# opensatelliteproject/xritdemod

Hardware: AMD Instinct MI355X
Metric: Msamples/s in -> soft-symbols/s out (LRIT 293 ksym/s chain); % HBM roofline (higher is better)
Workload: dtype f32

## Files before the change

### xritdemod_amd/csrc/agc.hip

```cpp
#include "kernels.h"

#include <cstdlib>
#include "scan.h"
#include "agc_wave.h"
#include "exact_walk.h"

namespace xrit {

struct AgcScanF {
    typedef AgcMap T;
    const float2 *x;
    float2 *y;
    const float *state_in;
    float *state_out;
    float rate, ref, maxg;
    long long n;
    int vec;

    __device__ T identity() const { return agc_identity(); }
    __device__ T combine(const T &lo, const T &hi) const { return agc_compose(lo, hi); }
    __device__ T reduce_run(long long i0, int cnt) const
    {
        T m = agc_identity();
        bool bad = false;
// ... 18 lines not shown
    {
        float g = agc_apply(pre, state_in[0]);
        if (cnt == SCAN_IPT && vec) {
            const float4 *xp = reinterpret_cast<const float4 *>(x + i0);
            float4 a = xp[0], b = xp[1], oa, ob;
            agc_step(a.x, a.y, g, rate, ref, maxg, oa.x, oa.y);
            agc_step(a.z, a.w, g, rate, ref, maxg, oa.z, oa.w);
            agc_step(b.x, b.y, g, rate, ref, maxg, ob.x, ob.y);
            agc_step(b.z, b.w, g, rate, ref, maxg, ob.z, ob.w);
            float4 *yp = reinterpret_cast<float4 *>(y + i0);
            yp[0] = oa;
            yp[1] = ob;
        } else {
            for (int k = 0; k < cnt; ++k) {
                float2 v = x[i0 + k];
                float yr, yi;
                agc_step(v.x, v.y, g, rate, ref, maxg, yr, yi);
                y[i0 + k] = make_float2(yr, yi);
            }
        }
        if (i0 + cnt == n) state_out[0] = g;
    }
};

__global__ void agc_serial_kernel(const float2 *x, float2 *y, const float *state_in, float *state_out,
                                  float rate, float ref, float maxg, long long n, int force)
{
    if (blockIdx.x != 0 || threadIdx.x != 0) return;
    if (!force && state_out[1] == 0.0f) return;
    float g = state_in[0];
    for (long long i = 0; i < n; ++i) {
        float2 v = x[i];
        float yr, yi;
        agc_step(v.x, v.y, g, rate, ref, maxg, yr, yi);
        y[i] = make_float2(yr, yi);
    }
    state_out[0] = g;
    state_out[1] = 2.0f;
}

__global__ void agc_begin_kernel(float *state_out)
{
    state_out[1] = 0.0f;
}

int AgcStage::init(float rate_, float reference, float gain0_, float max_gain)
{
    rate = rate_;
    ref = reference;
    maxg = max_gain;
    gain0 = gain0_;
    {
        int cus = 0, dev = 0;
        if (hipGetDevice(&dev) == hipSuccess && hipDeviceGetAttribute(&cus, hipDeviceAttributeMultiprocessorCount, dev) == hipSuccess && cus > 0)
            ex_walkers = 8 * cus;
        if (const char *e = getenv("XRIT_CX_WALKERS")) { const int v = atoi(e); if (v > 0) ex_walkers = v; }
        if (const char *e = getenv("XRIT_CX_MODE")) ex_mode = atoi(e) & 3;
    }
    XR_TRY(state.reserve(4 * sizeof(float)));
    float h[4] = {gain0_, 0.0f, gain0_, 0.0f};
    XR_HIP(hipMemcpy(state.p, h, sizeof h, hipMemcpyHostToDevice));
    if (!h_flag) XR_HIP(hipHostMalloc((void **)&h_flag, 64));
    *h_flag = 0.0f;
    cur = 0;
    return XRIT_OK;
}

__global__ void agc_reset_kernel(float *st, float g)
{
    st[0] = g; st[1] = 0.f; st[2] = g; st[3] = 0.f;
}

int AgcStage::reset(hipStream_t s)
{
    hipLaunchKernelGGL(agc_reset_kernel, dim3(1), dim3(1), 0, s, state.as<float>(), gain0);
    cur = 0;
    return XRIT_OK;
}

void AgcStage::release()
{
    state.release();
    aggs.release();
    joints.release();
    if (h_flag) { (void)hipHostFree(h_flag); h_flag = nullptr; }
}

int AgcStage::request_flag_at(const float *flag, hipStream_t s)
{
    XR_HIP(hipMemcpyAsync(h_flag, flag, sizeof(float), hipMemcpyDeviceToHost, s));
    return XRIT_OK;
}

int AgcStage::request_flag(hipStream_t s)
{
    XR_HIP(hipMemcpyAsync(h_flag, state.as<float>() + 2 * cur + 1, sizeof(float), hipMemcpyDeviceToHost, s));
    return XRIT_OK;
}

int AgcStage::run(const float2 *in, float2 *out, size_t n, hipStream_t s, Profiler *prof, bool use_exact)
{
    if (exact || use_exact) return run_exact(in, out, n, s, prof);
    if (n == 0) return XRIT_OK;
    float *sin_ = state.as<float>() + 2 * cur;
    float *sout = state.as<float>() + 2 * (cur ^ 1);
    int nb = scan_blocks((long long)n);
    XR_TRY(aggs.reserve((size_t)(nb + scan_blocks(nb) + 4) * sizeof(AgcMap)));
    const int vec = (((uintptr_t)in | (uintptr_t)out) & 15) == 0;
    AgcScanF f{in, out, sin_, sout, rate, ref, maxg, (long long)n, vec};
    {
        ProfScope ps(prof, "agc_reduce", s);
        hipLaunchKernelGGL(agc_begin_kernel, dim3(1), dim3(1), 0, s, sout);
        hipLaunchKernelGGL(scan_reduce_kernel<AgcScanF>, dim3(nb), dim3(SCAN_BLOCK), 0, s, f, (long long)n,
                           aggs.as<AgcMap>());
    }
    {
        ProfScope ps(prof, "agc_scan", s);
        scan_aggs_launch(f, aggs.as<AgcMap>(), nb, s);
    }
    {
        ProfScope ps(prof, "agc_apply", s);
        hipLaunchKernelGGL(scan_apply_kernel<AgcScanF>, dim3(nb), dim3(SCAN_BLOCK), 0, s, f, (long long)n,
                           aggs.as<AgcMap>());
        hipLaunchKernelGGL(agc_serial_kernel, dim3(1), dim3(1), 0, s, in, out, sin_, sout, rate, ref, maxg,
                           (long long)n, 0);
    }
    XR_HIP(hipGetLastError());
    cur ^= 1;
    return XRIT_OK;
}


constexpr int AGC_EX_WARM = 12288;
constexpr int AGC_EX_ROUNDS = 3;

__device__ __forceinline__ void agc_step_exact(float xr, float xi, float &g, float rate, float ref, float maxg, float &yr, float &yi)
{
    yr = xr * g;
    yi = xi * g;
    g += rate * (ref - ::sqrtf(yr * yr + yi * yi));
    if (maxg > 0.0f && g > maxg) g = maxg;
}

__device__ __forceinline__ float agx_scan(float d, float g0, float maxg, int mode, unsigned *lat)
{
    const int lane = threadIdx.x & 63;
    float gv = g0;
    if (mode & 2) {
        float gb = g0;
        int s = 0, seg = 0;
        bool done = false;
        for (; seg < 4 && !done; ++seg) {
            const bool in = lane >= s;
            const int og = xw::ord(gb);
            const int dG = in ? xw::ord(gb + d) - og : 0;
            const int S = xw::prefix(dG);
            const float gnext = xw::inv(og + S), gown = xw::inv(og + S - dG);
            float lg = gown + d;
            if (maxg > 0.0f && lg > maxg) lg = maxg;
            const unsigned long long bad = __builtin_amdgcn_ballot_w64(in && __float_as_uint(lg) != __float_as_uint(gnext));
            const int k = bad ? (int)__builtin_ctzll(bad) : 64;
            if (in && lane <= k) gv = gown;
            if (k >= 63) { done = true; break; }
            gb = xw::lane_of(lg, k);
            s = k + 1;
        }
// ... 88 lines not shown
    XR_TRY(aggs.reserve((size_t)(nb + scan_blocks(nb) + 4) * sizeof(AgcMap)));
    XR_TRY(joints.reserve((size_t)3 * W * sizeof(float2) + ((n >> 6) + 2) * sizeof(float2) + xw::NCNT * sizeof(unsigned)));
    AgcScanF f{in, out, sin_, sout, rate, ref, maxg, (long long)n, 0};
    {
        ProfScope ps(prof, "agc_reduce", s);
        hipLaunchKernelGGL(agc_begin_kernel, dim3(1), dim3(1), 0, s, sout);
        hipLaunchKernelGGL(scan_reduce_kernel<AgcScanF>, dim3(nb), dim3(SCAN_BLOCK), 0, s, f, (long long)n, aggs.as<AgcMap>());
    }
    {
        ProfScope ps(prof, "agc_scan", s);
        scan_aggs_launch(f, aggs.as<AgcMap>(), nb, s);
    }
    {
        ProfScope ps(prof, "agc_exact", s);
        xw::KArgs<AgcWalk> K{};
        xw::Args &A = K.a;
        A.x = in; A.y = out;
        A.js = joints.as<float2>(); A.je = A.js + W; A.used = A.je + W;
        A.bs = A.used + W;
        A.cnt = reinterpret_cast<unsigned *>(A.bs + (n >> 6) + 2);
        ex_cnt = A.cnt;
        A.n = (long long)n; A.Lw = (int)lw; A.H = AGC_EX_WARM; A.W = W;
        A.mode = ex_mode; A.prio = 1;
        K.p = AgcWalk::Par{aggs.as<AgcMap>(), sin_, sout, rate, ref, maxg};
        hipLaunchKernelGGL(xw::zero_kernel<AgcWalk>, dim3(1), dim3(64), 0, s, A.cnt, xw::NCNT);
        hipLaunchKernelGGL(xw::main_kernel<AgcWalk>, dim3(W), dim3(64), 0, s, K);
        hipLaunchKernelGGL(xw::used_kernel<AgcWalk>, dim3(div_up((size_t)W, 256)), dim3(256), 0, s, A);
        if (W > 1) {
            for (int r = 0; r < AGC_EX_ROUNDS; ++r) hipLaunchKernelGGL(xw::fix_kernel<AgcWalk>, dim3(W - 1), dim3(64), 0, s, K, 0);
            hipLaunchKernelGGL(xw::zero_kernel<AgcWalk>, dim3(1), dim3(64), 0, s, A.cnt, 1);
            hipLaunchKernelGGL(xw::fix_kernel<AgcWalk>, dim3(W - 1), dim3(64), 0, s, K, 1);
            hipLaunchKernelGGL(agc_exact_flag_kernel, dim3(1), dim3(1), 0, s, A.cnt, sout);
        }
        hipLaunchKernelGGL(agc_serial_exact_kernel, dim3(1), dim3(1), 0, s, in, out, sin_, sout, rate, ref, maxg, (long long)n);
    }
    XR_HIP(hipGetLastError());
    cur ^= 1;
    return XRIT_OK;
}

struct AgcRunF {
    typedef AgcMap T;
    __device__ T identity() const { return agc_identity(); }
    __device__ T combine(const T &lo, const T &hi) const { return agc_compose(lo, hi); }
};

template <int PL>
__global__ void __launch_bounds__(256) agc_apply_runs_kernel(const float2 *__restrict__ x, float2 *__restrict__ y,
                                                             const AgcMap *__restrict__ pre_run,
                                                             const float *__restrict__ state_in,
                                                             float *__restrict__ state_out, float rate, float ref,
                                                             float maxg, long long n)
{
    const int lane = threadIdx.x & 63;
    const long long run = (long long)blockIdx.x * 4 + (threadIdx.x >> 6);
    const long long i0 = run * (64 * PL) + (long long)lane * PL;
    int cnt = 0;
    if (i0 < n) cnt = (int)((n - i0) < PL ? (n - i0) : PL);
    float2 v[PL];
#pragma unroll
    for (int k = 0; k < PL; ++k) v[k] = k < cnt ? x[i0 + k] : make_float2(0.f, 0.f);
    AgcMap m = agc_identity();
#pragma unroll
    for (int k = 0; k < PL; ++k)
        if (k < cnt) m = agc_compose(m, agc_sample_map(v[k].x, v[k].y, rate, ref, maxg));
    const AgcMap ex = agc_wave_exclusive(m);
    if (cnt == 0) return;
    float g = agc_apply(agc_compose(pre_run[run], ex), state_in[0]);
#pragma unroll
    for (int k = 0; k < PL; ++k) {
        if (k < cnt) {
            float yr, yi;
            agc_step(v[k].x, v[k].y, g, rate, ref, maxg, yr, yi);
            y[i0 + k] = make_float2(yr, yi);
        }
    }
    if (i0 + cnt == n) state_out[0] = g;
}

constexpr int AGC_RUNS_PER_WAVE = 4;
template <int PL>
__global__ void __launch_bounds__(256) agc_run_maps_kernel(const float2 *__restrict__ x, AgcMap *__restrict__ maps,
                                                           float *__restrict__ state_out, float rate, float ref,
                                                           float maxg, long long n)
{
    const int lane = threadIdx.x & 63;
    const long long run0 = ((long long)blockIdx.x * 4 + (threadIdx.x >> 6)) * AGC_RUNS_PER_WAVE;
    float2 v[AGC_RUNS_PER_WAVE][PL];
#pragma unroll
    for (int r = 0; r < AGC_RUNS_PER_WAVE; ++r) {
        const long long i0 = (run0 + r) * (64 * PL) + (long long)lane * PL;
#pragma unroll
        for (int k = 0; k < PL; ++k) v[r][k] = x[min(i0 + k, n - 1)];
    }
    bool bad = false;
#pragma unroll
    for (int r = 0; r < AGC_RUNS_PER_WAVE; ++r) {
        const long long run = run0 + r;
        if (run * (64 * PL) >= n) break;
        const long long i0 = run * (64 * PL) + (long long)lane * PL;
        int cnt = 0;
        if (i0 < n) cnt = (int)((n - i0) < PL ? (n - i0) : PL);
        AgcMap m = agc_identity();
#pragma unroll
        for (int k = 0; k < PL; ++k) {
            if (k < cnt) {
                const AgcMap e = agc_sample_map(v[r][k].x, v[r][k].y, rate, ref, maxg);
                bad |= !(e.a >= 0.0f);
                m = agc_compose(m, e);
            }
        }
        m = agc_wave_total(m);
        if (lane == 0) maps[run] = m;
    }
    if (bad) state_out[1] = 1.0f;
}

int AgcStage::fused_reduce(const float2 *in, size_t n, int per_lane, hipStream_t s, Profiler *prof)
{
    AgcEpilogue epi{};
    XR_TRY(fused_begin(n, per_lane, s, &epi));
    if (n == 0) return XRIT_OK;
    if (per_lane != 3) { set_error("AGC: unsupported run shape %d", per_lane); return XRIT_E_INVALID; }
    const size_t rl = (size_t)64 * per_lane;
    const unsigned nr = div_up(n, rl);
    ProfScope ps(prof, "agc_reduce", s);
    hipLaunchKernelGGL(agc_run_maps_kernel<3>, dim3(div_up((size_t)nr, 4 * AGC_RUNS_PER_WAVE)), dim3(256), 0, s, in, epi.maps, epi.state_out,
                       rate, ref, maxg, (long long)n);
    XR_HIP(hipGetLastError());
    return XRIT_OK;
}

int AgcStage::fused_begin(size_t n, int per_lane, hipStream_t s, AgcEpilogue *epi)
{
    const size_t rl = (size_t)64 * per_lane;
    const int nr = (int)((n + rl - 1) / rl);
    XR_TRY(aggs.reserve((size_t)(nr + scan_blocks(nr) + 8) * sizeof(AgcMap)));
    float *sout = state.as<float>() + 2 * (cur ^ 1);
    hipLaunchKernelGGL(agc_begin_kernel, dim3(1), dim3(1), 0, s, sout);
    epi->maps = aggs.as<AgcMap>();
    epi->state_out = sout;
    epi->rate = rate;
    epi->ref = ref;
    epi->maxg = maxg;
    return XRIT_OK;
}

int AgcStage::fused_finish(const float2 *in, float2 *out, size_t n, int per_lane, hipStream_t s, Profiler *prof)
{
    if (n == 0) return XRIT_OK;
    float *sin_ = state.as<float>() + 2 * cur;
    float *sout = state.as<float>() + 2 * (cur ^ 1);
    const size_t rl = (size_t)64 * per_lane;
    const int nr = (int)((n + rl - 1) / rl);
    {
        ProfScope ps(prof, "agc_scan", s);
        scan_aggs_launch(AgcRunF{}, aggs.as<AgcMap>(), nr, s);
    }
    {
        ProfScope ps(prof, "agc_apply", s);
        const dim3 grid(div_up((size_t)nr, 4));
#define XR_AGC_APPLY(PL)                                                                                        \
    hipLaunchKernelGGL(agc_apply_runs_kernel<PL>, grid, dim3(256), 0, s, in, out, aggs.as<AgcMap>(), sin_, sout, \
                       rate, ref, maxg, (long long)n)
        switch (per_lane) {
        case 1: XR_AGC_APPLY(1); break;
        case 2: XR_AGC_APPLY(2); break;
        case 3: XR_AGC_APPLY(3); break;
        case 4: XR_AGC_APPLY(4); break;
        case 5: XR_AGC_APPLY(5); break;
        default: set_error("AGC: unsupported run shape %d", per_lane); return XRIT_E_INVALID;
        }
#undef XR_AGC_APPLY
        hipLaunchKernelGGL(agc_serial_kernel, dim3(1), dim3(1), 0, s, in, out, sin_, sout, rate, ref, maxg,
                           (long long)n, 0);
    }
    XR_HIP(hipGetLastError());
    cur ^= 1;
    return XRIT_OK;
}

int AgcStage::fused_scan(const float2 *in, float2 *fallback, size_t n, int per_lane, hipStream_t s, Profiler *prof,
                         AgcFill *fill)
{
    float *sin_ = state.as<float>() + 2 * cur;
    float *sout = state.as<float>() + 2 * (cur ^ 1);
    const size_t rl = (size_t)64 * per_lane;
    const int nr = (int)((n + rl - 1) / rl);
    {
        ProfScope ps(prof, "agc_scan", s);
        if (nr > 0) scan_aggs_launch(AgcRunF{}, aggs.as<AgcMap>(), nr, s);
        hipLaunchKernelGGL(agc_serial_kernel, dim3(1), dim3(1), 0, s, in, fallback, sin_, sout, rate, ref, maxg,
                           (long long)n, 0);
    }
    XR_HIP(hipGetLastError());
    fill->x = in;
    fill->pre_run = aggs.as<AgcMap>();
    fill->state_in = sin_;
    fill->state_out = sout;
    fill->rate = rate;
    fill->ref = ref;
    fill->maxg = maxg;
    fill->per_lane = per_lane;
    cur ^= 1;
    return XRIT_OK;
}

int AgcStage::exact_counters(unsigned *out8, hipStream_t s)
{
    for (int i = 0; i < 8; ++i) out8[i] = 0;
    if (!ex_cnt) return XRIT_OK;
    XR_HIP(hipMemcpyAsync(out8, ex_cnt, 8 * sizeof(unsigned), hipMemcpyDeviceToHost, s));
    XR_HIP(hipStreamSynchronize(s));
    return XRIT_OK;
}

int AgcStage::gain(float *g, hipStream_t s)
{
    XR_HIP(hipMemcpyAsync(g, state.as<float>() + 2 * cur, sizeof(float), hipMemcpyDeviceToHost, s));
    XR_HIP(hipStreamSynchronize(s));
    return XRIT_OK;
}

int AgcStage::fallback_flag(float *flag, hipStream_t s)
{
    XR_HIP(hipMemcpyAsync(flag, state.as<float>() + 2 * cur + 1, sizeof(float), hipMemcpyDeviceToHost, s));
    XR_HIP(hipStreamSynchronize(s));
    return XRIT_OK;
}

}
```

### xritdemod_amd/csrc/agc_wave.h

```cpp
#pragma once

#include <hip/hip_runtime.h>

#include "loop_core.h"

namespace xrit {

template <int CTRL> __device__ __forceinline__ float agc_dpp(float fill, float v)
{
    return __int_as_float(__builtin_amdgcn_update_dpp(__float_as_int(fill), __float_as_int(v), CTRL, 0xf, 0xf, false));
}

template <int SH> __device__ __forceinline__ AgcMap agc_row_shr(const AgcMap &v)
{
    AgcMap r;
    r.a = agc_dpp<0x110 + SH>(1.0f, v.a);
    r.b = agc_dpp<0x110 + SH>(0.0f, v.b);
    r.c = agc_dpp<0x110 + SH>(INFINITY, v.c);
    return r;
}

__device__ __forceinline__ AgcMap agc_row_scan(AgcMap v)
{
    v = agc_compose(agc_row_shr<1>(v), v);
    v = agc_compose(agc_row_shr<2>(v), v);
    v = agc_compose(agc_row_shr<4>(v), v);
    v = agc_compose(agc_row_shr<8>(v), v);
    return v;
}

__device__ __forceinline__ AgcMap agc_read_lane(const AgcMap &v, int lane)
{
    AgcMap r;
    r.a = __int_as_float(__builtin_amdgcn_readlane(__float_as_int(v.a), lane));
    r.b = __int_as_float(__builtin_amdgcn_readlane(__float_as_int(v.b), lane));
    r.c = __int_as_float(__builtin_amdgcn_readlane(__float_as_int(v.c), lane));
    return r;
}

__device__ __forceinline__ AgcMap agc_wave_total(const AgcMap &v)
{
    const AgcMap s = agc_row_scan(v);
    AgcMap t = agc_read_lane(s, 15);
    t = agc_compose(t, agc_read_lane(s, 31));
    t = agc_compose(t, agc_read_lane(s, 47));
    t = agc_compose(t, agc_read_lane(s, 63));
    return t;
}

__device__ __forceinline__ AgcMap agc_wave_exclusive(const AgcMap &v)
{
    const AgcMap s = agc_row_scan(v);
    const AgcMap t0 = agc_read_lane(s, 15), t1 = agc_read_lane(s, 31), t2 = agc_read_lane(s, 47);
    const int row = (threadIdx.x & 63) >> 4;
    AgcMap pre = agc_identity();
    if (row >= 1) pre = t0;
    if (row >= 2) pre = agc_compose(pre, t1);
    if (row >= 3) pre = agc_compose(pre, t2);
    return agc_compose(pre, agc_row_shr<1>(s));
}

}
```

### xritdemod_amd/csrc/demod.cpp

```cpp
#include "kernels.h"

#include <chrono>
#include <cmath>
#include <mutex>
#include <new>
#include <thread>
#include <vector>

namespace xrit {

static thread_local char g_err[512] = "";

void set_error(const char *fmt, ...)
{
    va_list ap;
    va_start(ap, fmt);
    vsnprintf(g_err, sizeof g_err, fmt, ap);
    va_end(ap);
}
const char *get_error() { return g_err; }

int select_device(int device)
{
    int count = 0;
// ... 347 lines not shown
    for (auto w : d->stream3) XR_HIP(hipStreamSynchronize(w));
    if (d->costas.job.n && d->pf_count > 0) {
        for (int i = 0; i < d->pf_count; ++i)
            if (d->pf[i].costas_begun && !d->pf[i].costas_finished) { bool redone = false; (void)d->costas.finish(d->pf[i].c_stream ? d->pf[i].c_stream : d->stream2, nullptr, &redone); }
    }
    d->pf_count = 0;
    d->last_fe_set = -1;
    XR_TRY(d->dec.reset(s));
    XR_TRY(d->rrc.reset(s));
    XR_TRY(d->agc.reset(s));
    XR_TRY(d->rtl.reset(s));
    XR_TRY(d->costas.reset(s));
    XR_TRY(d->clock.reset(s));
    d->poisoned = false;
    return XRIT_OK;
}

int xrit_build_experiments(void)
{
#ifdef XRIT_EXPERIMENTS
    return 1;
#else
    return 0;
#endif
}

void *xrit_demod_stream(xrit_demod *d) { return d ? (void *)d->stream : nullptr; }
float xrit_demod_sps(const xrit_demod *d) { return d ? d->sps : 0.f; }
int xrit_demod_decimator_ntaps(const xrit_demod *d) { return d ? d->dec_ntaps : 0; }

static int keep_stage(xrit_demod *d, int idx, const void *src, size_t n, hipStream_t s)
{
    if (!d->keep_stages) return XRIT_OK;
    XR_TRY(d->stage_buf[idx].reserve((n + 1) * sizeof(float2)));
    if (n) XR_HIP(hipMemcpyAsync(d->stage_buf[idx].p, src, n * sizeof(float2), hipMemcpyDeviceToDevice, s));
    d->stage_n[idx] = n;
    return XRIT_OK;
}

struct SliceIO {
    size_t length = 0;
    const float2 *rrc = nullptr;
    bool stat_ready = false;
    int set = 0;
    const float *agc_flag = nullptr;
    bool exact = false;
};

static bool front_exact_call(const xrit_demod *d, size_t n)
{
    if (d->cfg.front_exact == 2) return true;
    if (d->cfg.front_exact != 0) return false;
    const unsigned D = d->cfg.decimation;
    const double length = (double)(D > 1 ? n / D : n);
    return length / (double)d->sps < (double)d->clock.ov_min;
}

int xrit_demod_front_exact_for(const xrit_demod *d, size_t n)
{
    if (!d) return XRIT_E_INVALID;
    return front_exact_call(d, n) ? 1 : 0;
}

static int front_end(xrit_demod *d, const void *in, size_t n, int type, int set, hipStream_t s, Profiler *prof, SliceIO *io)
{
    io->set = set;
    const bool ex = front_exact_call(d, n);
    io->exact = ex;
    const unsigned D = d->cfg.decimation;
    if (type == XRIT_SAMPLE_U8IQ) {
        XR_TRY(d->bufR[set].reserve((n + 8) * sizeof(float2)));
        XR_TRY(d->rtl.run(in, d->bufR[set].as<float2>(), n, s, prof));
        in = d->bufR[set].p;
        type = XRIT_SAMPLE_FLOATIQ;
    }
    size_t length = n;
    if (D > 1) length = n / D;
    io->length = length;
    XR_TRY(d->bufA[set].reserve((length + 8) * sizeof(float2)));
    XR_TRY(d->bufB[set].reserve((length + 8) * sizeof(float2)));
    float2 *A = d->bufA[set].as<float2>(), *B = d->bufB[set].as<float2>();
    const float2 *cur = nullptr;
    const bool agc_fused = !ex && D > 1 && length > 0 && d->dec.agc_supported();
    if (D > 1) {
        AgcEpilogue epi{};
        if (agc_fused) XR_TRY(d->agc.fused_begin(length, d->dec.RC, s, &epi));
        XR_TRY(d->dec.run(in, type, A, length, s, prof, nullptr, 0, agc_fused ? &epi : nullptr, nullptr, ex));
        cur = A;
    } else if (type != XRIT_SAMPLE_FLOATIQ) {
        ProfScope ps(prof, "convert", s);
        XR_TRY(launch_convert(in, type, A, length, s));
        cur = A;
    } else {
        cur = reinterpret_cast<const float2 *>(in);
    }
    XR_TRY(keep_stage(d, 0, cur, length, s));
    const bool agc_in_rrc = agc_fused && !d->keep_stages && d->rrc.agc_fill_supported(d->dec.RC);
    const bool agc_in_rrc_d1 = !ex && !agc_fused && length > 0 && !d->keep_stages && d->rrc.agc_fill_supported(3);
    AgcFill fill{};
    float2 *Cfb = nullptr;
    if (agc_in_rrc || agc_in_rrc_d1) {
        XR_TRY(d->bufC[set].reserve((length + 8) * sizeof(float2)));
        Cfb = d->bufC[set].as<float2>();
        if (agc_in_rrc_d1) XR_TRY(d->agc.fused_reduce(cur, length, 3, s, prof));
        XR_TRY(d->agc.fused_scan(cur, Cfb, length, agc_in_rrc ? d->dec.RC : 3, s, prof, &fill));
    }
    else if (agc_fused) XR_TRY(d->agc.fused_finish(cur, B, length, d->dec.RC, s, prof));
    else XR_TRY(d->agc.run(cur, B, length, s, prof, ex));
    XR_TRY(keep_stage(d, 1, B, length, s));
    constexpr int SUB = 8;
    XR_TRY(d->stat[set].reserve(((length + SUB - 1) / SUB + 2) * sizeof(float2)));
    io->stat_ready = length > 0 && d->rrc.stat_supported(SUB) && d->costas.L % SUB == 0;
    const bool fill_on = agc_in_rrc || agc_in_rrc_d1;
    float2 *rrc_out = fill_on ? B : A;
    XR_TRY(d->rrc.run(fill_on ? Cfb : B, XRIT_SAMPLE_FLOATIQ, rrc_out, length, s, prof, io->stat_ready ? d->stat[set].as<float2>() : nullptr, SUB,
                      nullptr, fill_on ? &fill : nullptr, ex));
    XR_TRY(keep_stage(d, 2, rrc_out, length, s));
    io->rrc = rrc_out;
    io->agc_flag = d->agc.state.as<float>() + 2 * d->agc.cur + 1;
    return XRIT_OK;
}

static bool ov_call(xrit_demod *d, size_t n);

static int launch_prefetched(xrit_demod *d, xrit_demod::Prefetched &f, hipEvent_t after)
{
    XR_HIP(hipStreamWaitEvent(d->stream2, d->ev_ready, 0));
    if (after) XR_HIP(hipStreamWaitEvent(d->stream2, after, 0));
    if (d->last_fe_set >= 0) XR_HIP(hipStreamWaitEvent(d->stream2, d->ev_fe[d->last_fe_set], 0));
    const int set = d->next_set;
    d->next_set ^= 1;
    SliceIO io;
    Profiler *prof = d->prof.enabled ? &d->prof : nullptr;
    d->dec.prio = d->rrc.prio = ov_call(d, f.n) ? 1 : 0;
    int rc = front_end(d, f.samples, f.n, f.type, set, d->stream2, prof, &io);
    d->dec.prio = d->rrc.prio = 0;
    if (rc != XRIT_OK) { d->poisoned = true; return rc; }
    XR_HIP(hipEventRecord(d->ev_fe[set], d->stream2));
    d->last_fe_set = set;
    f.set = set;
    f.length = io.length; f.rrc = io.rrc; f.stat_ready = io.stat_ready; f.agc_flag = io.agc_flag; f.exact = io.exact;
    f.launched = true;
    return XRIT_OK;
}

static int costas_enqueue(xrit_demod *d, const SliceIO &io, hipStream_t s, Profiler *prof, float2 **slot_out)
{
    const size_t length = io.length;
    const int L = d->costas.L;
    float2 *slot = nullptr;
    XR_TRY(d->clock.input_slot(length, &slot, s));
    double2 *om = nullptr;
    if (length) om = d->clock.om_slot((int)((length + (size_t)L - 1) / (size_t)L), L);
    const double inv_sps = 1.0 / (double)d->sps;
    const float2 *stat = io.stat_ready ? d->stat[io.set].as<float2>() : nullptr;
    XR_TRY(d->costas.begin(io.rrc, slot, length, s, prof, stat, om, 0, inv_sps, io.exact));
    if (length) XR_TRY(d->clock.om_scan(s));
    if (length) XR_TRY(d->agc.request_flag_at(io.agc_flag, s));
    *slot_out = slot;
    return XRIT_OK;
}

static void set_relay_hook(xrit_demod *d, hipStream_t s)
{
    d->clock.before_relay = [d, s](int phase) -> int {
        if (phase == 0) {
            if (d->pf_count > 0 && !d->pf[0].launched) XR_HIP(hipEventRecord(d->ev_relay, s));
            return XRIT_OK;
        }
        if (d->pf_count > 0 && !d->pf[0].launched) {
            if (d->clock.trace_env) fprintf(stderr, "[xrit] the registered front end starts with the relay kernels%s\n", d->costas_idle ? ", its Costas loop behind it" : "");
            XR_TRY(launch_prefetched(d, d->pf[0], d->ev_relay));
            if (d->costas_idle) {
                xrit_demod::Prefetched &f = d->pf[0];
                SliceIO io;
                io.length = f.length; io.rrc = f.rrc; io.stat_ready = f.stat_ready; io.set = f.set; io.agc_flag = f.agc_flag; io.exact = f.exact;
                int rc = costas_enqueue(d, io, d->stream2, d->prof.enabled ? &d->prof : nullptr, &f.slot);
                if (rc != XRIT_OK) { d->poisoned = true; return rc; }
                XR_HIP(hipEventRecord(d->ev_costas, d->stream2));
                f.costas_begun = true;
// ... 872 lines not shown
```

### xritdemod_amd/csrc/fir.hip

```cpp
#include "kernels.h"

#include <cstdlib>
#include <new>
#include "agc_wave.h"

namespace xrit {

template <int TYPE> struct SampleLoad;
template <> struct SampleLoad<XRIT_SAMPLE_FLOATIQ> {
    static __device__ __forceinline__ float2 at(const void *p, size_t j) { return reinterpret_cast<const float2 *>(p)[j]; }
};
template <> struct SampleLoad<XRIT_SAMPLE_S16IQ> {
    static __device__ __forceinline__ float2 at(const void *p, size_t j)
    {
        short2 v = reinterpret_cast<const short2 *>(p)[j];
        return make_float2(v.x / 32768.f, v.y / 32768.f);
    }
};
template <> struct SampleLoad<XRIT_SAMPLE_S8IQ> {
    static __device__ __forceinline__ float2 at(const void *p, size_t j)
    {
        char2 v = reinterpret_cast<const char2 *>(p)[j];
        return make_float2(v.x / 128.f, v.y / 128.f);
    }
};

template <int APL>
__device__ __forceinline__ void fir_fill_through_agc(float2 *tile, const AgcFill &af, const float2 *__restrict__ hist,
                                                     int T, long long tile_start, int tile_len, long long n_in)
{
    constexpr int RL = 64 * APL;
    constexpr int MAXIT = 3;
    const int tid = threadIdx.x, nthr = blockDim.x;
    const int wave = tid >> 6, lane = tid & 63, nwaves = nthr >> 6;
    const long long t_end = tile_start + tile_len < n_in ? tile_start + tile_len : n_in;
    const long long first_run = (tile_start > 0 ? tile_start : 0) / RL;
    float2 v[MAXIT][APL];
    int cnt[MAXIT];
#pragma unroll
    for (int it = 0; it < MAXIT; ++it) {
        const long long rr = first_run + wave + (long long)it * nwaves;
        const long long i0 = rr * RL + (long long)lane * APL;
        cnt[it] = 0;
        if (rr * RL < t_end && i0 < n_in) cnt[it] = (int)((n_in - i0) < APL ? (n_in - i0) : APL);
#pragma unroll
        for (int k = 0; k < APL; ++k) v[it][k] = k < cnt[it] ? af.x[i0 + k] : make_float2(0.f, 0.f);
    }
    const float g0 = af.state_in[0];
#pragma unroll
    for (int it = 0; it < MAXIT; ++it) {
        const long long rr = first_run + wave + (long long)it * nwaves;
        if (rr * RL >= t_end) break;
        AgcMap m = agc_identity();
#pragma unroll
        for (int k = 0; k < APL; ++k)
            if (k < cnt[it]) m = agc_compose(m, agc_sample_map(v[it][k].x, v[it][k].y, af.rate, af.ref, af.maxg));
        const AgcMap ex = agc_wave_exclusive(m);
        float gg = agc_apply(agc_compose(af.pre_run[rr], ex), g0);
        const long long i0 = rr * RL + (long long)lane * APL;
#pragma unroll
        for (int k = 0; k < APL; ++k) {
            if (k < cnt[it]) {
                float yr, yi;
                agc_step(v[it][k].x, v[it][k].y, gg, af.rate, af.ref, af.maxg, yr, yi);
                const long long idx = i0 + k - tile_start;
                if (idx >= 0 && idx < tile_len) tile[idx] = make_float2(yr, yi);
                if (i0 + k == n_in - 1) af.state_out[0] = gg;
            }
        }
    }
    for (int idx = tid; idx < tile_len; idx += nthr) {
        const long long j = tile_start + idx;
        if (j < 0) {
            const long long hj = (T - 1) + j;
            tile[idx] = hj >= 0 ? hist[hj] : make_float2(0.f, 0.f);
        } else if (j >= n_in) {
            tile[idx] = make_float2(0.f, 0.f);
        }
    }
}

template <int TYPE>
__device__ __forceinline__ void fir_leave_history(const void *__restrict__ in, const float2 *__restrict__ hist_old,
                                                  float2 *__restrict__ hist_new, int T, long long n_in)
{
    for (int i = threadIdx.x; i < T - 1; i += blockDim.x) {
        const long long j = n_in - (T - 1) + i;
        float2 v;
        if (j >= 0) v = SampleLoad<TYPE>::at(in, (size_t)j);
        else {
            const long long hj = (T - 1) + j;
            v = hj >= 0 ? hist_old[hj] : make_float2(0.f, 0.f);
        }
        hist_new[i] = v;
    }
}

template <bool MF> __device__ __forceinline__ int fir_mf_pos(int q) { return MF ? q + 20 * (q / 80) : q; }

#ifndef XRIT_FE_PRIO
#define XRIT_FE_PRIO 1
#endif
template <int RC, bool PAD, int TYPE, int APL = 0, int TS = 0, int DS = 1, bool MF = false, bool EX = false>
__global__ void __launch_bounds__(256)
fir_decim_kernel(const void *__restrict__ in, const float2 *__restrict__ hist, float2 *__restrict__ out,
                 const float *__restrict__ g, int T, int D, int Wpad, long long n_out, long long n_in,
                 int tile_len, float2 *__restrict__ stat, int statL, AgcEpilogue agc, AgcFill af,
                 float2 *__restrict__ hist_new, const float *__restrict__ mfb = nullptr)
{
    if (statL >> 16) __builtin_amdgcn_s_setprio(XRIT_FE_PRIO);
    statL &= 0xffff;
    if (hist_new != nullptr && blockIdx.x == gridDim.x - 1 && (APL == 0 || af.state_out[1] != 0.0f))
        fir_leave_history<TYPE>(in, hist, hist_new, T, n_in);
    extern __shared__ __attribute__((aligned(16))) char smem_raw[];
    float2 *tile = reinterpret_cast<float2 *>(smem_raw);
    const int nthr = blockDim.x;
    const int tid = threadIdx.x;
    const long long OB = (long long)nthr * RC;
    const long long out_base = (long long)blockIdx.x * OB;
    const long long tile_start = out_base * D - (T - 1);

    if (APL > 0 && af.state_out[1] == 0.0f) {
        fir_fill_through_agc<(APL > 0 ? APL : 1)>(tile, af, hist, T, tile_start, tile_len, n_in);
    } else if (tile_start >= 0 && tile_start + tile_len <= n_in) {
        int idx = tid;
        if (TYPE == XRIT_SAMPLE_FLOATIQ && !PAD && !MF && (tile_start & 1) == 0 &&
            (reinterpret_cast<size_t>(in) & 15) == 0) {
            const float4 *in4 = reinterpret_cast<const float4 *>(reinterpret_cast<const float2 *>(in) + tile_start);
            float4 *tile4 = reinterpret_cast<float4 *>(tile);
            const int pairs = tile_len >> 1;
            int p = tid;
#ifndef XRIT_NO_LDS_DIRECT
            for (; p - (tid & 63) < pairs; p += nthr) {
                if (p < pairs)
                    __builtin_amdgcn_global_load_lds((const __attribute__((address_space(1))) void *)(in4 + p),
                                                     (__attribute__((address_space(3))) void *)(tile4 + (p - (tid & 63))), 16, 0, 0);
            }
            asm volatile("s_waitcnt vmcnt(0)" ::: "memory");
#endif
#define XR_TILE_BATCH4(U)                                                                   \
    for (; p + (U - 1) * nthr < pairs; p += U * nthr) {                                     \
        float4 v[U];                                                                        \
        _Pragma("unroll") for (int u = 0; u < U; ++u) v[u] = in4[p + u * nthr];             \
        _Pragma("unroll") for (int u = 0; u < U; ++u) tile4[p + u * nthr] = v[u];           \
    }
            XR_TILE_BATCH4(8)
            XR_TILE_BATCH4(4)
            XR_TILE_BATCH4(2)
            XR_TILE_BATCH4(1)
#undef XR_TILE_BATCH4
            idx = 2 * pairs + tid;
        }
#define XR_TILE_BATCH(U)                                                                                      \
    for (; idx + (U - 1) * nthr < tile_len; idx += U * nthr) {                                               \
        float2 v[U];                                                                                          \
        _Pragma("unroll") for (int u = 0; u < U; ++u)                                                         \
            v[u] = SampleLoad<TYPE>::at(in, (size_t)(tile_start + idx + u * nthr));                           \
        _Pragma("unroll") for (int u = 0; u < U; ++u) {                                                       \
            const int q = idx + u * nthr;                                                                     \
            tile[PAD ? q + q / D : fir_mf_pos<MF>(q)] = v[u];                                                 \
        }                                                                                                     \
    }
        XR_TILE_BATCH(8)
        XR_TILE_BATCH(4)
        XR_TILE_BATCH(2)
        XR_TILE_BATCH(1)
#undef XR_TILE_BATCH
    } else {
        for (int idx = tid; idx < tile_len; idx += nthr) {
            long long j = tile_start + idx;
            float2 v = make_float2(0.f, 0.f);
            if (j < 0) {
                long long hj = (T - 1) + j;
                if (hj >= 0) v = hist[hj];
            } else if (j < n_in) {
                v = SampleLoad<TYPE>::at(in, (size_t)j);
            }
            int pos = PAD ? idx + idx / D : fir_mf_pos<MF>(idx);
            tile[pos] = v;
        }
    }
    __syncthreads();
    if (APL > 0 && hist_new != nullptr && blockIdx.x == gridDim.x - 1 && af.state_out[1] == 0.0f) {
        for (int i = tid; i < T - 1; i += nthr) hist_new[i] = tile[(int)(n_in - (T - 1) + i - tile_start)];
    }

    float2 acc[RC];
#pragma unroll
    for (int c = 0; c < RC; ++c) acc[c] = make_float2(0.f, 0.f);

    const int lane_base = PAD ? tid * RC * (D + 1) : tid * RC * D;
    const float2 *w = tile + lane_base;
    if (MF) {
#ifdef XRIT_EXPERIMENTS
#include "../../experiments/csrc/fir_mfma_dec.inc"
#endif
    } else if (TS > 0) {
        typedef float v2f __attribute__((ext_vector_type(2)));
        constexpr int NP = (TS + 1) / 2;
        const unsigned long long *gp = reinterpret_cast<const unsigned long long *>(g);
        unsigned long long tp[NP > 0 ? NP : 1];
#pragma unroll
        for (int k = 0; k < NP; ++k) tp[k] = gp[k];
        v2f a[RC];
#pragma unroll
        for (int c = 0; c < RC; ++c) a[c] = (v2f){0.f, 0.f};
// ... 54 lines not shown
                float2 x = w[off + k];
#pragma unroll
                for (int c = 0; c < RC; ++c) {
                    float tp = g[c * Wpad + i + k];
                    acc[c].x = fmaf(tp, x.x, acc[c].x);
                    acc[c].y = fmaf(tp, x.y, acc[c].y);
                }
            }
            i += run;
            off += D + 1;
        }
    } else if (EX) {
        typedef float v2f __attribute__((ext_vector_type(2)));
        v2f a[RC][4];
#pragma unroll
        for (int c = 0; c < RC; ++c)
#pragma unroll
            for (int j = 0; j < 4; ++j) a[c][j] = (v2f){0.f, 0.f};
        for (int i = 0; i < Wpad; i += 4) {
            const float2 q0 = w[i], q1 = w[i + 1], q2 = w[i + 2], q3 = w[i + 3];
            const v2f x0 = {q0.x, q0.y}, x1 = {q1.x, q1.y}, x2 = {q2.x, q2.y}, x3 = {q3.x, q3.y};
#pragma unroll
            for (int c = 0; c < RC; ++c) {
                const float *gc = g + c * Wpad + i;
                const float t0 = gc[0], t1 = gc[1], t2 = gc[2], t3 = gc[3];
                const v2f p0 = x0 * t0, p1 = x1 * t1, p2 = x2 * t2, p3 = x3 * t3;
                a[c][0] = a[c][0] + p0;
                a[c][1] = a[c][1] + p1;
                a[c][2] = a[c][2] + p2;
                a[c][3] = a[c][3] + p3;
            }
        }
#pragma unroll
        for (int c = 0; c < RC; ++c) {
            const int sh = (c * D) & 3;
            v2f r;
            if (sh == 0) r = (a[c][0] + a[c][1]) + (a[c][2] + a[c][3]);
            else if (sh == 1) r = (a[c][1] + a[c][2]) + (a[c][3] + a[c][0]);
            else if (sh == 2) r = (a[c][2] + a[c][3]) + (a[c][0] + a[c][1]);
            else r = (a[c][3] + a[c][0]) + (a[c][1] + a[c][2]);
            acc[c] = make_float2(r.x, r.y);
        }
    } else {
        for (int i = 0; i < Wpad; i += 4) {
            float2 x0 = w[i], x1 = w[i + 1], x2 = w[i + 2], x3 = w[i + 3];
#pragma unroll
            for (int c = 0; c < RC; ++c) {
                const float *gc = g + c * Wpad + i;
                float t0 = gc[0], t1 = gc[1], t2 = gc[2], t3 = gc[3];
                acc[c].x = fmaf(t0, x0.x, acc[c].x);
                acc[c].y = fmaf(t0, x0.y, acc[c].y);
                acc[c].x = fmaf(t1, x1.x, acc[c].x);
                acc[c].y = fmaf(t1, x1.y, acc[c].y);
                acc[c].x = fmaf(t2, x2.x, acc[c].x);
                acc[c].y = fmaf(t2, x2.y, acc[c].y);
                acc[c].x = fmaf(t3, x3.x, acc[c].x);
                acc[c].y = fmaf(t3, x3.y, acc[c].y);
            }
        }
    }
    const long long m0 = out_base + (long long)tid * RC;
    {
        __syncthreads();
        float2 *ot = tile;
#pragma unroll
        for (int c = 0; c < RC; ++c) ot[tid * RC + c] = acc[c];
        __syncthreads();
        const long long left = n_out - out_base;
        const int cnt = left < OB ? (int)left : (int)OB;
        for (int k = tid; k < cnt; k += nthr) out[out_base + k] = ot[k];
    }
    if (!PAD && agc.maps != nullptr) {
        AgcMap v = agc_identity();
        bool bad = false;
#pragma unroll
        for (int c = 0; c < RC; ++c) {
            if (m0 + c < n_out) {
                AgcMap e = agc_sample_map(acc[c].x, acc[c].y, agc.rate, agc.ref, agc.maxg);
                bad |= !(e.a >= 0.0f);
                v = agc_compose(v, e);
            }
        }
        if (bad) agc.state_out[1] = 1.0f;
        v = agc_wave_total(v);
        const int lane = tid & 63;
        if (lane == 0 && m0 < n_out) agc.maps[m0 / (64 * RC)] = v;
    }
    if (stat != nullptr) {
        const float2 *ot = tile;
        if (statL == 8) {
            for (int i = tid; i < (int)OB; i += nthr) {
                const long long o = out_base + i;
                float sr = 0.f, si = 0.f;
                if (o < n_out) {
                    const float2 z = ot[i];
                    sr = z.x * z.x - z.y * z.y;
                    si = 2.0f * z.x * z.y;
                }
                sr += __int_as_float(__builtin_amdgcn_update_dpp(0, __float_as_int(sr), 0x111, 0xf, 0xf, true));
                si += __int_as_float(__builtin_amdgcn_update_dpp(0, __float_as_int(si), 0x111, 0xf, 0xf, true));
                sr += __int_as_float(__builtin_amdgcn_update_dpp(0, __float_as_int(sr), 0x112, 0xf, 0xf, true));
                si += __int_as_float(__builtin_amdgcn_update_dpp(0, __float_as_int(si), 0x112, 0xf, 0xf, true));
                sr += __int_as_float(__builtin_amdgcn_update_dpp(0, __float_as_int(sr), 0x114, 0xf, 0xf, true));
                si += __int_as_float(__builtin_amdgcn_update_dpp(0, __float_as_int(si), 0x114, 0xf, 0xf, true));
                if ((tid & 7) == 7 && o - 7 < n_out) stat[o >> 3] = make_float2(sr, si);
            }
        } else {
            const int runs = (int)(OB / statL);
            const int wave = tid >> 6, lane = tid & 63, nwaves = nthr >> 6;
            for (int j = wave; j < runs; j += nwaves) {
                const long long first = out_base + (long long)j * statL;
                if (first >= n_out) break;
                float sr = 0.f, si = 0.f;
                for (int i = lane; i < statL; i += 64) {
                    if (first + i < n_out) {
                        const float2 z = ot[j * statL + i];
                        sr += z.x * z.x - z.y * z.y;
                        si += 2.0f * z.x * z.y;
                    }
                }
                for (int off = 32; off > 0; off >>= 1) {
                    sr += __shfl_down(sr, off, 64);
                    si += __shfl_down(si, off, 64);
                }
                if (lane == 0) stat[first / statL] = make_float2(sr, si);
            }
        }
    }
}

#ifndef XRIT_POLY_THREADS
#define XRIT_POLY_THREADS 256
#endif
template <int DP, int PR, int NQ, int TYPE>
__global__ void __launch_bounds__(XRIT_POLY_THREADS)
fir_poly_kernel(const void *__restrict__ in, const float2 *__restrict__ hist, float2 *__restrict__ out,
                const float *__restrict__ hq , int T, long long n_out, long long n_in, int tile_len,
                float2 *__restrict__ hist_new)
{
    if (hist_new != nullptr && blockIdx.x == 0) fir_leave_history<TYPE>(in, hist, hist_new, T, n_in);
    extern __shared__ __attribute__((aligned(16))) char smem_raw[];
    float2 *tile = reinterpret_cast<float2 *>(smem_raw);
    const int tid = threadIdx.x, nthr = blockDim.x;
    const int OB = (nthr / DP) * PR;
    const unsigned per = gridDim.x >> 3;
    const long long tb = (long long)(blockIdx.x & 7) * per + (blockIdx.x >> 3);
    const long long out_base = tb * OB;
    if (out_base >= n_out) return;
    const long long tile_start = out_base * DP - (long long)(NQ * DP);

    if (TYPE == XRIT_SAMPLE_FLOATIQ && tile_start >= 0 && tile_start + tile_len <= n_in && (tile_start & 1) == 0 &&
        (reinterpret_cast<size_t>(in) & 15) == 0) {
        const float4 *in4 = reinterpret_cast<const float4 *>(reinterpret_cast<const float2 *>(in) + tile_start);
        float4 *tile4 = reinterpret_cast<float4 *>(tile);
        const int pairs = tile_len >> 1;
        constexpr int UF = (((NQ + (XRIT_POLY_THREADS / DP) * PR - 1) * DP + 2) / 2 + XRIT_POLY_THREADS - 1) / XRIT_POLY_THREADS;
#ifndef XRIT_NO_LDS_DIRECT
        for (int p = tid; p - (tid & 63) < pairs; p += nthr)
            if (p < pairs)
                __builtin_amdgcn_global_load_lds((const __attribute__((address_space(1))) void *)(in4 + p),
                                                 (__attribute__((address_space(3))) void *)(tile4 + (p - (tid & 63))), 16, 0, 0);
        asm volatile("s_waitcnt vmcnt(0)" ::: "memory");
        for (int p0 = pairs + tid; p0 < pairs; p0 += UF * nthr) {
#else
        for (int p0 = tid; p0 < pairs; p0 += UF * nthr) {
#endif
            float4 v[UF];
#pragma unroll
// ... 533 lines not shown
```

### xritdemod_amd/csrc/kernels.h

```cpp
#pragma once

#include <functional>

#include "common.h"
#include "loop_core.h"
#include "taps.h"

namespace xrit {

struct FirStage {
    int T = 0, D = 1, RC = 3, W = 0, Wpad = 0, threads = 256, tile_len = 0, cur = 0;
    bool pad = false;
    bool mfma_dec = false;
    bool no_static_dec = false, no_static_mf = false;
    int prio = 0;
    bool poly = false;
    bool exact = false, ex_pad = false;
    int ex_threads = 256, ex_opt = 2, ex_tile_len = 0;
    size_t ex_lds = 0;
    DevBuf rt;
    std::vector<float> taps_host;
    int set_exact(bool on);
#ifndef XRIT_POLY_PR
#define XRIT_POLY_PR 16
#endif
    static constexpr int POLY_PR = XRIT_POLY_PR, POLY_NQ = 32;
    size_t lds_bytes = 0;
    DevBuf g;
    DevBuf mfb;
    DevBuf hist[2];
    int init(const float *taps, int ntaps, int decim);
    int reset(hipStream_t s);
    void release();
    int run(const void *in, int sample_type, float2 *out, size_t n_out, hipStream_t s, Profiler *prof,
            float2 *stat = nullptr, int statL = 0, const struct AgcEpilogue *agc = nullptr,
            const struct AgcFill *fill = nullptr, bool use_exact = false);
    FirStage *twin = nullptr;
    bool last_twin = false;
    FirStage() = default;
    FirStage(const FirStage &) = delete;
    FirStage &operator=(const FirStage &) = delete;
    bool agc_fill_supported(int per_lane) const;
    bool stat_supported(int statL) const;
    bool agc_supported() const;
};

constexpr int AGC_RUN_MAX_PER_LANE = 5;
struct AgcFill {
    const float2 *x;
    const struct AgcMap *pre_run;
    const float *state_in;
    float *state_out;
    float rate, ref, maxg;
    int per_lane;
};
struct AgcEpilogue {
    struct AgcMap *maps;
    float *state_out;
    float rate, ref, maxg;
};

struct RtlIngestStage {
    float alpha = 0;
    DevBuf state;
    DevBuf aggs;
    int cur = 0;
    int init(float sample_rate);
    int reset(hipStream_t s);
    void release();
    int run(const void *in_u8, float2 *out, size_t n_complex, hipStream_t s, Profiler *prof);
};

struct AgcStage {
    float rate = 0, ref = 0, maxg = 0;
    DevBuf state;
    DevBuf aggs;
    int cur = 0;
    int init(float rate, float reference, float gain, float max_gain);
    int reset(hipStream_t s);
    float gain0 = 1.0f;
    void release();
    int run(const float2 *in, float2 *out, size_t n, hipStream_t s, Profiler *prof, bool use_exact = false);
    bool exact = false;
    DevBuf joints;
    int ex_walkers = 2048, ex_mode = 3;
    int run_exact(const float2 *in, float2 *out, size_t n, hipStream_t s, Profiler *prof);
    unsigned *ex_cnt = nullptr;
    int exact_counters(unsigned *out8, hipStream_t s);
    int fused_begin(size_t n, int per_lane, hipStream_t s, AgcEpilogue *epi);
    int fused_finish(const float2 *in, float2 *out, size_t n, int per_lane, hipStream_t s, Profiler *prof);
    int fused_reduce(const float2 *in, size_t n, int per_lane, hipStream_t s, Profiler *prof);
    int fused_scan(const float2 *in, float2 *fallback, size_t n, int per_lane, hipStream_t s, Profiler *prof, AgcFill *fill);
    int gain(float *g, hipStream_t s);
    int fallback_flag(float *flag, hipStream_t s);
    int request_flag(hipStream_t s);
    int request_flag_at(const float *flag, hipStream_t s);
    float requested_flag() const { return h_flag ? *h_flag : 0.0f; }
    float *h_flag = nullptr;
};

struct CostasStage {
    CostasGains gains{};
    int L = 256;
    int max_passes = 32;
    float trust = 1.0f, tol_phase = 1e-5f, tol_freq = 3e-8f;
    DevBuf state;
    DevBuf S, E, J, stat, sub, dlin, work, flags, counters, wsolve, rescue;
    bool model_step = true;
    float model_accept = 5e-3f;
    bool force_gated = false;
    int final_warm = 0;
    bool keep_spare = false, trace_env = false, no_serial_walk = false;
    int rescue_after = 32;
    long long rescue_max_samples = 4 << 20;
    unsigned rescues = 0;
    bool walked = false;
    int serial_rescue(hipStream_t s, Profiler *prof);
    unsigned *h_counters = nullptr;
    int cur = 0;
    int passes = 0;
    unsigned unconverged = 0;
    float max_residual = 0;
    int init(float loop_bw, int chain_len, int max_passes);
    int reset(hipStream_t s);
    void release();
    int run(const float2 *in, float2 *out, size_t n, hipStream_t s, Profiler *prof, const float2 *sub_ext = nullptr,
            double2 *om = nullptr, long long om_off = 0, double inv_sps = 0.0);
    int begin(const float2 *in, float2 *out, size_t n, hipStream_t s, Profiler *prof, const float2 *sub_ext,
              double2 *om, long long om_off, double inv_sps, bool use_exact = false);
    bool closed() const;
    int finish(hipStream_t s, Profiler *prof, bool *redone);
    int enqueue_passes(int count, hipStream_t s, Profiler *prof);
    int enqueue_final(hipStream_t s, Profiler *prof);
    struct Job {
        const float2 *in = nullptr; float2 *out = nullptr; size_t n = 0; int K = 0; int enqueued = 0;
        double2 *om = nullptr; long long om_off = 0; double inv_sps = 0;
        bool gated = false;
        bool rescued = false;
        bool exact = false;
        float model_accept = 0;
    } job;
    int batch = 4;
    int stable = 0, last_passes = -1;
    int get_state(float *phase, float *freq, hipStream_t s);
    bool exact = false;
    int ex_mode = 3;
    int ex_hist = -1;
    int ex_prio = 1;
    int ex_walkers = 2048;
    DevBuf xj, xbs, xcnt;
    unsigned *h_xcnt = nullptr;
    int ex_W = 0, ex_rounds = 0;
    bool ex_args_valid = false;
    unsigned ex_open = 0, ex_nonconverged = 0;
    unsigned long long ex_blocks = 0, ex_picard = 0, ex_segs = 0, ex_fallbacks = 0;
    int exact_plan(size_t n, int *Lw, int *W, int *H) const;
    int enqueue_exact(hipStream_t s, Profiler *prof);
    int finish_exact(hipStream_t s, Profiler *prof, bool *redone);
    int flip_phase(hipStream_t s);
};

int launch_loop_sincosf(const float *d_x, float *d_sin, float *d_cos, size_t n, hipStream_t s);

struct ClockStage {
    ClockPar par{};
    float sps = 0, mu0 = 0.5f;
    int NS = 64;
    int cu_count = 256;
    long long lds_per_cu = 160 * 1024;
    bool auto_ns = true;
    bool serial = false;
    int max_passes = 48, min_passes = 4;
// ... 184 lines not shown
```

Before: 154,300.

## Store per-lane AGC exclusive prefixes in reduce pass and reuse in RRC fill

The reduce pass (decimator epilogue or run-maps kernel) now keeps the intra-wave row scan and writes each lane's exclusive prefix map to a new per-run buffer. The AGC-through-RRC fill path then loads these prefixes instead of recomputing per-sample AGC maps and a second wave scan. This trades recomputing transcendental-heavy sample maps for extra HBM traffic: 768 bytes per run written and read back, plus a new buffer allocation. The agc_in_rrc decision is moved earlier so the buffer is only produced when the fill path will consume it.

```diff
diff --git a/xritdemod_amd/csrc/agc.hip b/xritdemod_amd/csrc/agc.hip
--- a/xritdemod_amd/csrc/agc.hip
+++ b/xritdemod_amd/csrc/agc.hip
@@ -124,6 +124,8 @@
 {
     state.release();
     aggs.release();
+    lane_ex.release();
+    lane_ex_ready = false;
     joints.release();
     if (h_flag) { (void)hipHostFree(h_flag); h_flag = nullptr; }
 }
@@ -378,7 +380,7 @@
 template <int PL>
 __global__ void __launch_bounds__(256) agc_run_maps_kernel(const float2 *__restrict__ x, AgcMap *__restrict__ maps,
                                                            float *__restrict__ state_out, float rate, float ref,
-                                                           float maxg, long long n)
+                                                           float maxg, long long n, float *__restrict__ lane_ex)
 {
     const int lane = threadIdx.x & 63;
     const long long run0 = ((long long)blockIdx.x * 4 + (threadIdx.x >> 6)) * AGC_RUNS_PER_WAVE;
@@ -406,7 +408,9 @@
                 m = agc_compose(m, e);
             }
         }
-        m = agc_wave_total(m);
+        const AgcMap sc = agc_row_scan(m);
+        if (lane_ex != nullptr) agc_store_lane_ex(lane_ex + run * AGC_LANE_EX, agc_wave_exclusive_of_scan(sc), lane);
+        m = agc_wave_total_of_scan(sc);
         if (lane == 0) maps[run] = m;
     }
     if (bad) state_out[1] = 1.0f;
@@ -415,23 +419,25 @@
 int AgcStage::fused_reduce(const float2 *in, size_t n, int per_lane, hipStream_t s, Profiler *prof)
 {
     AgcEpilogue epi{};
-    XR_TRY(fused_begin(n, per_lane, s, &epi));
+    XR_TRY(fused_begin(n, per_lane, s, &epi, true));
     if (n == 0) return XRIT_OK;
     if (per_lane != 3) { set_error("AGC: unsupported run shape %d", per_lane); return XRIT_E_INVALID; }
     const size_t rl = (size_t)64 * per_lane;
     const unsigned nr = div_up(n, rl);
     ProfScope ps(prof, "agc_reduce", s);
     hipLaunchKernelGGL(agc_run_maps_kernel<3>, dim3(div_up((size_t)nr, 4 * AGC_RUNS_PER_WAVE)), dim3(256), 0, s, in, epi.maps, epi.state_out,
-                       rate, ref, maxg, (long long)n);
+                       rate, ref, maxg, (long long)n, epi.lane_ex);
     XR_HIP(hipGetLastError());
     return XRIT_OK;
 }
 
-int AgcStage::fused_begin(size_t n, int per_lane, hipStream_t s, AgcEpilogue *epi)
+int AgcStage::fused_begin(size_t n, int per_lane, hipStream_t s, AgcEpilogue *epi, bool want_lane_ex)
 {
     const size_t rl = (size_t)64 * per_lane;
     const int nr = (int)((n + rl - 1) / rl);
     XR_TRY(aggs.reserve((size_t)(nr + scan_blocks(nr) + 8) * sizeof(AgcMap)));
+    if (want_lane_ex) XR_TRY(lane_ex.reserve((size_t)nr * AGC_LANE_EX * sizeof(float)));
+    lane_ex_ready = want_lane_ex;
     float *sout = state.as<float>() + 2 * (cur ^ 1);
     hipLaunchKernelGGL(agc_begin_kernel, dim3(1), dim3(1), 0, s, sout);
     epi->maps = aggs.as<AgcMap>();
@@ -439,6 +445,7 @@
     epi->rate = rate;
     epi->ref = ref;
     epi->maxg = maxg;
+    epi->lane_ex = want_lane_ex ? lane_ex.as<float>() : nullptr;
     return XRIT_OK;
 }
 
@@ -498,6 +505,7 @@
     fill->ref = ref;
     fill->maxg = maxg;
     fill->per_lane = per_lane;
+    fill->lane_ex = lane_ex_ready ? lane_ex.as<float>() : nullptr;
     cur ^= 1;
     return XRIT_OK;
 }
diff --git a/xritdemod_amd/csrc/agc_wave.h b/xritdemod_amd/csrc/agc_wave.h
--- a/xritdemod_amd/csrc/agc_wave.h
+++ b/xritdemod_amd/csrc/agc_wave.h
@@ -38,9 +38,8 @@
     return r;
 }
 
-__device__ __forceinline__ AgcMap agc_wave_total(const AgcMap &v)
+__device__ __forceinline__ AgcMap agc_wave_total_of_scan(const AgcMap &s)
 {
-    const AgcMap s = agc_row_scan(v);
     AgcMap t = agc_read_lane(s, 15);
     t = agc_compose(t, agc_read_lane(s, 31));
     t = agc_compose(t, agc_read_lane(s, 47));
@@ -48,9 +47,10 @@
     return t;
 }
 
-__device__ __forceinline__ AgcMap agc_wave_exclusive(const AgcMap &v)
+__device__ __forceinline__ AgcMap agc_wave_total(const AgcMap &v) { return agc_wave_total_of_scan(agc_row_scan(v)); }
+
+__device__ __forceinline__ AgcMap agc_wave_exclusive_of_scan(const AgcMap &s)
 {
-    const AgcMap s = agc_row_scan(v);
     const AgcMap t0 = agc_read_lane(s, 15), t1 = agc_read_lane(s, 31), t2 = agc_read_lane(s, 47);
     const int row = (threadIdx.x & 63) >> 4;
     AgcMap pre = agc_identity();
@@ -60,4 +60,18 @@
     return agc_compose(pre, agc_row_shr<1>(s));
 }
 
+__device__ __forceinline__ AgcMap agc_wave_exclusive(const AgcMap &v) { return agc_wave_exclusive_of_scan(agc_row_scan(v)); }
+
+__device__ __forceinline__ void agc_store_lane_ex(float *run_ex, const AgcMap &e, int lane)
+{
+    run_ex[lane] = e.a;
+    run_ex[64 + lane] = e.b;
+    run_ex[128 + lane] = e.c;
 }
+
+__device__ __forceinline__ AgcMap agc_load_lane_ex(const float *__restrict__ run_ex, int lane)
+{
+    return AgcMap{run_ex[lane], run_ex[64 + lane], run_ex[128 + lane]};
+}
+
+}
diff --git a/xritdemod_amd/csrc/demod.cpp b/xritdemod_amd/csrc/demod.cpp
--- a/xritdemod_amd/csrc/demod.cpp
+++ b/xritdemod_amd/csrc/demod.cpp
@@ -453,9 +453,10 @@
     float2 *A = d->bufA[set].as<float2>(), *B = d->bufB[set].as<float2>();
     const float2 *cur = nullptr;
     const bool agc_fused = !ex && D > 1 && length > 0 && d->dec.agc_supported();
+    const bool agc_in_rrc = agc_fused && !d->keep_stages && d->rrc.agc_fill_supported(d->dec.RC);
     if (D > 1) {
         AgcEpilogue epi{};
-        if (agc_fused) XR_TRY(d->agc.fused_begin(length, d->dec.RC, s, &epi));
+        if (agc_fused) XR_TRY(d->agc.fused_begin(length, d->dec.RC, s, &epi, agc_in_rrc));
         XR_TRY(d->dec.run(in, type, A, length, s, prof, nullptr, 0, agc_fused ? &epi : nullptr, nullptr, ex));
         cur = A;
     } else if (type != XRIT_SAMPLE_FLOATIQ) {
@@ -466,7 +467,6 @@
         cur = reinterpret_cast<const float2 *>(in);
     }
     XR_TRY(keep_stage(d, 0, cur, length, s));
-    const bool agc_in_rrc = agc_fused && !d->keep_stages && d->rrc.agc_fill_supported(d->dec.RC);
     const bool agc_in_rrc_d1 = !ex && !agc_fused && length > 0 && !d->keep_stages && d->rrc.agc_fill_supported(3);
     AgcFill fill{};
     float2 *Cfb = nullptr;
diff --git a/xritdemod_amd/csrc/fir.hip b/xritdemod_amd/csrc/fir.hip
--- a/xritdemod_amd/csrc/fir.hip
+++ b/xritdemod_amd/csrc/fir.hip
@@ -25,7 +25,7 @@
     }
 };
 
-template <int APL>
+template <int APL, bool LEX>
 __device__ __forceinline__ void fir_fill_through_agc(float2 *tile, const AgcFill &af, const float2 *__restrict__ hist,
                                                      int T, long long tile_start, int tile_len, long long n_in)
 {
@@ -36,6 +36,7 @@
     const long long t_end = tile_start + tile_len < n_in ? tile_start + tile_len : n_in;
     const long long first_run = (tile_start > 0 ? tile_start : 0) / RL;
     float2 v[MAXIT][APL];
+    AgcMap lex[MAXIT];
     int cnt[MAXIT];
 #pragma unroll
     for (int it = 0; it < MAXIT; ++it) {
@@ -45,17 +46,22 @@
         if (rr * RL < t_end && i0 < n_in) cnt[it] = (int)((n_in - i0) < APL ? (n_in - i0) : APL);
 #pragma unroll
         for (int k = 0; k < APL; ++k) v[it][k] = k < cnt[it] ? af.x[i0 + k] : make_float2(0.f, 0.f);
+        lex[it] = agc_identity();
+        if (LEX && cnt[it] > 0) lex[it] = agc_load_lane_ex(af.lane_ex + rr * AGC_LANE_EX, lane);
     }
     const float g0 = af.state_in[0];
 #pragma unroll
     for (int it = 0; it < MAXIT; ++it) {
         const long long rr = first_run + wave + (long long)it * nwaves;
         if (rr * RL >= t_end) break;
-        AgcMap m = agc_identity();
-#pragma unroll
-        for (int k = 0; k < APL; ++k)
-            if (k < cnt[it]) m = agc_compose(m, agc_sample_map(v[it][k].x, v[it][k].y, af.rate, af.ref, af.maxg));
-        const AgcMap ex = agc_wave_exclusive(m);
+        AgcMap ex = lex[it];
+        if (!LEX) {
+            AgcMap m = agc_identity();
+#pragma unroll
+            for (int k = 0; k < APL; ++k)
+                if (k < cnt[it]) m = agc_compose(m, agc_sample_map(v[it][k].x, v[it][k].y, af.rate, af.ref, af.maxg));
+            ex = agc_wave_exclusive(m);
+        }
         float gg = agc_apply(agc_compose(af.pre_run[rr], ex), g0);
         const long long i0 = rr * RL + (long long)lane * APL;
 #pragma unroll
@@ -121,7 +127,8 @@
     const long long tile_start = out_base * D - (T - 1);
 
     if (APL > 0 && af.state_out[1] == 0.0f) {
-        fir_fill_through_agc<(APL > 0 ? APL : 1)>(tile, af, hist, T, tile_start, tile_len, n_in);
+        if (af.lane_ex != nullptr) fir_fill_through_agc<(APL > 0 ? APL : 1), true>(tile, af, hist, T, tile_start, tile_len, n_in);
+        else fir_fill_through_agc<(APL > 0 ? APL : 1), false>(tile, af, hist, T, tile_start, tile_len, n_in);
     } else if (tile_start >= 0 && tile_start + tile_len <= n_in) {
         int idx = tid;
         if (TYPE == XRIT_SAMPLE_FLOATIQ && !PAD && !MF && (tile_start & 1) == 0 &&
@@ -342,8 +349,13 @@
             }
         }
         if (bad) agc.state_out[1] = 1.0f;
-        v = agc_wave_total(v);
+        const AgcMap sc = agc_row_scan(v);
         const int lane = tid & 63;
+        if (agc.lane_ex != nullptr) {
+            const AgcMap ex = agc_wave_exclusive_of_scan(sc);
+            if (m0 - (long long)lane * RC < n_out) agc_store_lane_ex(agc.lane_ex + (m0 / (64 * RC)) * AGC_LANE_EX, ex, lane);
+        }
+        v = agc_wave_total_of_scan(sc);
         if (lane == 0 && m0 < n_out) agc.maps[m0 / (64 * RC)] = v;
     }
     if (stat != nullptr) {
diff --git a/xritdemod_amd/csrc/kernels.h b/xritdemod_amd/csrc/kernels.h
--- a/xritdemod_amd/csrc/kernels.h
+++ b/xritdemod_amd/csrc/kernels.h
@@ -53,11 +53,14 @@
     float *state_out;
     float rate, ref, maxg;
     int per_lane;
-};
+    const float *lane_ex;
+};
+constexpr int AGC_LANE_EX = 3 * 64;
 struct AgcEpilogue {
     struct AgcMap *maps;
     float *state_out;
     float rate, ref, maxg;
+    float *lane_ex;
 };
 
 struct RtlIngestStage {
@@ -75,6 +78,8 @@
     float rate = 0, ref = 0, maxg = 0;
     DevBuf state;
     DevBuf aggs;
+    DevBuf lane_ex;
+    bool lane_ex_ready = false;
     int cur = 0;
     int init(float rate, float reference, float gain, float max_gain);
     int reset(hipStream_t s);
@@ -87,7 +92,7 @@
     int run_exact(const float2 *in, float2 *out, size_t n, hipStream_t s, Profiler *prof);
     unsigned *ex_cnt = nullptr;
     int exact_counters(unsigned *out8, hipStream_t s);
-    int fused_begin(size_t n, int per_lane, hipStream_t s, AgcEpilogue *epi);
+    int fused_begin(size_t n, int per_lane, hipStream_t s, AgcEpilogue *epi, bool want_lane_ex = false);
     int fused_finish(const float2 *in, float2 *out, size_t n, int per_lane, hipStream_t s, Profiler *prof);
     int fused_reduce(const float2 *in, size_t n, int per_lane, hipStream_t s, Profiler *prof);
     int fused_scan(const float2 *in, float2 *fallback, size_t n, int per_lane, hipStream_t s, Profiler *prof, AgcFill *fill);
```

Result: no change. 153,900 (median of 6 runs) (-0.2%).
